# lanl-ansi/RestartSQP

Measured on NVIDIA B200. Metric: QP subproblems/sec, higher is better.
Workload: dtype f64

## Files before the change

restartsqp_b200/csrc/qp_kernel.cuh:

```cuda
#pragma once
#include <cuda_runtime.h>
#include <stdint.h>
#include "tma.cuh"

namespace sqpb200 {

#define QP_EPS 2.221e-16
#define QP_INFTY 1.0e20
#define QP_ZERO 1.0e-25
#define QP_BOUND_RELAX 1.0e4
#define QP_EPS_NUM (-1.0e3 * QP_EPS)
#define QP_EPS_DEN (1.0e3 * QP_EPS)
#define QP_EPS_FLIP (1.0e3 * QP_EPS)
#define QP_EPS_REG (1.0e3 * QP_EPS)
#define QP_EPS_LI (1.0e5 * QP_EPS)

enum { ST_OPTIMAL = 20, ST_INTERNAL = 21, ST_INFEASIBLE = 22, ST_UNBOUNDED = 23, ST_NOTINIT = 25, ST_HOMOTOPY = 28,
       ST_CAPACITY = 31  };
enum { MODE_COLD = 0, MODE_HOT_FIXED = 1, MODE_HOT_VARIED = 2,
       MODE_REINIT = 3  };
enum { FLAG_FLIPPING = 1, FLAG_RAMPING = 2, FLAG_DRIFT = 4, FLAG_KEEP_STATE = 8,
       FLAG_FORCE_GUESS = 16 ,
       FLAG_NO_CARRY = 32 ,
       FLAG_FLIP_AS_HOTSTART = 64  };
// ... 74 lines not shown
extern __shared__ __align__(128) double qp_smem[];

struct MinKey {
    double t;
    int pos;
};
__device__ __forceinline__ bool key_less(double t1, int p1, double t2, int p2) { return t1 < t2 || (t1 == t2 && p1 < p2); }

__device__ __forceinline__ double quot(double x, double d, double ri) {
    const double q0 = x * ri;
    const double r = __fma_rn(-q0, d, x);
    return __fma_rn(r, ri, q0);
}

#define QP_FN __noinline__
#ifndef QP_UNROLL_N
#define QP_UNROLL_N 1
#endif
#define QP_STR_(x) #x
#define QP_STR(x) QP_STR_(x)
#define QP_U1 _Pragma(QP_STR(unroll QP_UNROLL_N))
#ifdef QP_PROFILE
#define PROF_T0 long long prof_t0_ = clock64();
#define PROF_RESET prof_t0_ = clock64();
#define PROF2_T0 long long prof_t2_ = clock64();
#define PROF2_ADD(i) do { long long t_ = clock64(); if (lane == 0 && sA.prof) atomicAdd((unsigned long long*)&sA.prof[i], (unsigned long long)(t_ - prof_t2_)); prof_t2_ = t_; } while (0)
#define PROF_ADD(i) do { long long t_ = clock64(); if (lane == 0 && sA.prof) atomicAdd((unsigned long long*)&sA.prof[i], (unsigned long long)(t_ - prof_t0_)); prof_t0_ = t_; } while (0)
#else
#define PROF_T0
#define PROF_RESET
#define PROF2_T0
#define PROF2_ADD(i) do { } while (0)
#define PROF_ADD(i) do { } while (0)
#endif
enum { PR_STEPDIR = 0, PR_RATIO = 1, PR_STEP = 2, PR_REMOVE = 3, PR_EXTEND = 4, PR_WVEC = 5, PR_ADD = 6, PR_REFAC_W = 7, PR_REFAC_M = 8,
       PR_REFAC_CHOL = 9, PR_DRIFT = 10, PR_ENSURE_LI = 11, PR_RSOLVE = 12, PR_SETUP = 13, PR_EPILOGUE = 14, PR_TOTAL = 15 };

template <int TEAM> struct PatIdx { typedef int type; };
template <> struct PatIdx<32> { typedef short type; };
template <> struct PatIdx<16> { typedef short type; };
template <> struct PatIdx<8> { typedef short type; };
template <int TEAM> __device__ __forceinline__ unsigned team_mask() {
    if (TEAM >= 32) return 0xffffffffu;
    return ((1u << (TEAM & 31)) - 1u) << ((threadIdx.x & 31) & ~(TEAM - 1));
}
__shared__ double* sSlice;
__shared__ int sClusterSize;
__shared__ uint32_t sPhase;
__shared__ __align__(8) uint64_t sFull[3];
__shared__ double sRedT[32];
__shared__ int sRedP[32];

#define QP_CTX                                                                                     \
    const int lane = (TEAM <= 32) ? (int)(threadIdx.x & (TEAM - 1)) : (int)threadIdx.x;            \
    double* const slice = (TEAM <= 32) ? qp_smem + (size_t)(threadIdx.x / TEAM) * sA.slice_doubles : sSlice; \
    int* const hdr = reinterpret_cast<int*>(slice);                                                \
    const int nV = sA.nV, nC = sA.nC, ld = sA.ld, cap = sA.cap;                                    \
    (void)lane; (void)hdr; (void)nV; (void)nC; (void)ld; (void)cap;
#define QP_PAT                                                                                     \
    const pidx* const pat = (TEAM <= 32)                                                           \
        ? reinterpret_cast<const pidx*>(qp_smem + (size_t)(blockDim.x / TEAM) * sA.slice_doubles) \
        : reinterpret_cast<const pidx*>(sA.gpat);

#define V_(name) (slice + sA.o##name)
#define S_(k) (reinterpret_cast<short*>(slice + sA.oS) + (k))
#define sB_ S_(0)
#define FR_ S_(nV)
#define posFR_ S_(2 * nV)
#define sC_ S_(3 * nV)
#define AC_ S_(3 * nV + nC)
#define posAC_ S_(3 * nV + 2 * nC)
#define R_(a_, b_) RT[(a_) * ld + (b_)]
#define T_(i, j) RT[(cap - 1 - (i)) * ld + (j)]
#ifndef QP_DOT_UNROLL_N
#define QP_DOT_UNROLL_N 1
#endif
#define DOT_UNROLL _Pragma("unroll (TEAM <= 32 ? DOT_N_SMALL : 8)")
#define SYNC() do { if (TEAM <= 32) __syncwarp(team_mask<TEAM>()); else __syncthreads(); } while (0)

template <int TEAM>
struct QPT {
    static constexpr int DOT_N_SMALL = QP_DOT_UNROLL_N;
    typedef typename PatIdx<TEAM>::type pidx;
    static __device__ QP_FN void mulH(const double* v, double* out) {
        QP_CTX QP_PAT
        const pidx *Hp = pat + sA.pHp, *Hi = pat + sA.pHi;
        const double* Hv = V_(Hv);
        const bool has_H = sA.has_H && !sA.is_lp;
        const double reg = sA.is_lp ? QP_EPS_REG : 0.0;
        QP_U1 for (int c = lane; c < nV; c += TEAM) {
            double s = 0.0;
            if (has_H) {
                int e1 = Hp[c + 1];
                QP_U1 for (int e = Hp[c]; e < e1; e++) s += Hv[e] * v[Hi[e]];
            }
            if (reg != 0.0) s += reg * v[c];
            out[c] = s;
        }
        SYNC();
    }
    static __device__ QP_FN void mulH_noreg(const double* v, double* out) {
        QP_CTX QP_PAT
        const pidx *Hp = pat + sA.pHp, *Hi = pat + sA.pHi;
        const double* Hv = V_(Hv);
        const bool has_H = sA.has_H && !sA.is_lp;
        QP_U1 for (int c = lane; c < nV; c += TEAM) {
            double s = 0.0;
            if (has_H) {
                int e1 = Hp[c + 1];
                QP_U1 for (int e = Hp[c]; e < e1; e++) s += Hv[e] * v[Hi[e]];
            }
            out[c] = s;
        }
        SYNC();
    }
    static __device__ QP_FN void mulA(const double* v, double* out) {
        QP_CTX QP_PAT
        const pidx *Arp = pat + sA.pArp, *Aci = pat + sA.pAci, *Aperm = pat + sA.pAperm;
        const double* Av = V_(Av);
        QP_U1 for (int r = lane; r < nC; r += TEAM) {
            double s = 0.0;
            int k1 = Arp[r + 1];
            QP_U1 for (int k = Arp[r]; k < k1; k++) s += Av[Aperm[k]] * v[Aci[k]];
            out[r] = s;
        }
        SYNC();
    }
    static __device__ QP_FN void mulAT(const double* yc, double* out) {
        QP_CTX QP_PAT
        const pidx *Ap = pat + sA.pAp, *Ai = pat + sA.pAi;
        const double* Av = V_(Av);
        QP_U1 for (int c = lane; c < nV; c += TEAM) {
            double s = 0.0;
            int e1 = Ap[c + 1];
            QP_U1 for (int e = Ap[c]; e < e1; e++) s += Av[e] * yc[Ai[e]];
            out[c] = s;
        }
        SYNC();
    }
    static __device__ __forceinline__ double A_entry(const pidx* pat, const double* Av, int r, int c) {
        const pidx *Arp = pat + sA.pArp, *Aci = pat + sA.pAci, *Aperm = pat + sA.pAperm;
        double s = 0.0;
        int k1 = Arp[r + 1];
        QP_U1 for (int k = Arp[r]; k < k1; k++)
            if (Aci[k] == c) s += Av[Aperm[k]];
        return s;
    }

    static __device__ __forceinline__ MinKey team_min(double t, int pos) {
        const unsigned tm = team_mask<TEAM>();
        QP_U1 for (int o = (TEAM < 32 ? TEAM : 32) / 2; o > 0; o >>= 1) {
            double t2_ = __shfl_xor_sync(tm, t, o);
            int p2 = __shfl_xor_sync(tm, pos, o);
            if (key_less(t2_, p2, t, pos)) { t = t2_; pos = p2; }
        }
        if (TEAM > 32) {
            __syncthreads();
            if ((threadIdx.x & 31) == 0) { sRedT[threadIdx.x >> 5] = t; sRedP[threadIdx.x >> 5] = pos; }
            __syncthreads();
            t = sRedT[0]; pos = sRedP[0];
            QP_U1 for (int k = 1; k < TEAM / 32; k++)
                if (key_less(sRedT[k], sRedP[k], t, pos)) { t = sRedT[k]; pos = sRedP[k]; }
        }
        MinKey r; r.t = t; r.pos = pos;
        return r;
    }

    static __device__ __forceinline__ void givens(double a_, double b_, double& c, double& s, double& r) {
        if (a_ == 0.0) { c = 1.0; s = 0.0; r = b_; return; }
        double h = sqrt(a_ * a_ + b_ * b_);
        c = b_ / h; s = a_ / h; r = h;
    }

    static __device__ QP_FN void proj_column(int b) {
        QP_CTX
        double *t1 = V_(t1), *t2 = V_(t2);
        const double* Q = V_(Q);
        const short* posFR = posFR_;
        QP_U1 for (int i = lane; i < nV; i += TEAM) { int p = posFR[i]; t1[i] = (p >= 0) ? Q[p * ld + b] : 0.0; }
        SYNC();
        mulH(t1, t2);
    }
    static __device__ QP_FN int recompute_R() {
        QP_CTX
        const int nFR = hdr[0], nAC = hdr[1], nZ = nFR - nAC;
        if (nZ <= 0) return 0;
        double* RT = V_(RT);
        if (sA.is_lp) {
            double sr = sqrt(QP_EPS_REG);
            QP_U1 for (int k = lane; k < nZ * nZ; k += TEAM) { int a_ = k / nZ, b_ = k % nZ; R_(a_, b_) = (a_ == b_) ? sr : 0.0; }
#ifndef QP_EXACT
            if constexpr (TEAM > 32) {
                double* W = V_(W);
                for (int k = lane; k < nZ * 64; k += TEAM) { const int a_ = k >> 6, c_ = k & 63; if (c_ < ld) W[(size_t)a_ * ld + c_] = (c_ == (a_ & 63)) ? 1.0 / sr : 0.0; }
            }
#endif
            SYNC();
            return 0;
        }
        if constexpr (TEAM > 32) return recompute_R_blocked();
        PROF_T0
        {
            QP_PAT
            const double *Q = V_(Q), *Hv = V_(Hv);
            double* Wc = V_(t1);
            const short *FR = FR_, *posFR = posFR_;
            const pidx *Hp = pat + sA.pHp, *Hi = pat + sA.pHi;
            const bool has_H = sA.has_H != 0;
            int CH = sA.nW / nFR;
            if (CH > nZ) CH = nZ;
            QP_U1 for (int b0 = 0; b0 < nZ; b0 += CH) {
                const int cw = (nZ - b0 < CH) ? nZ - b0 : CH;
                QP_U1 for (int e = lane; e < nFR * cw; e += TEAM) {
                    const int p = e / cw, bb = e - p * cw;
                    double s = 0.0;
                    if (has_H) {
                        const int c = FR[p], e1 = Hp[c + 1];
                        QP_U1 for (int h = Hp[c]; h < e1; h++) {
                            const int pr = posFR[Hi[h]];
                            s += Hv[h] * ((pr >= 0) ? Q[pr * ld + b0 + bb] : 0.0);
// ... 1077 lines not shown

    static __device__ QP_FN void constraint_w(int c, double& wz2, double& a2) {
        QP_CTX QP_PAT
        const int nFR = hdr[0], nAC = hdr[1], nZ = nFR - nAC;
        double *a = V_(a), *w = V_(w);
        const double *Q = V_(Q), *Av = V_(Av);
        const short* FR = FR_;
        QP_U1 for (int p = lane; p < nFR; p += TEAM) a[p] = A_entry(pat, Av, c, FR[p]);
        SYNC();
#ifndef QP_EXACT
        if constexpr (TEAM > 32) {
            col_sums_auto(sA.oQ, nFR, 0, nFR, sA.oa, sA.ow, false);
            double s2p = 0.0, z2p = 0.0;
            for (int p = lane; p < nFR; p += TEAM) s2p += a[p] * a[p];
            for (int j = lane; j < nZ; j += TEAM) z2p += w[j] * w[j];
            a2 = team_sum(s2p); wz2 = team_sum(z2p);
            SYNC();
            return;
        }
#endif
        QP_U1 for (int j = lane; j < nFR; j += TEAM) {
            double s = 0.0;
            DOT_UNROLL for (int p = 0; p < nFR; p++) s += Q[p * ld + j] * a[p];
            w[j] = s;
        }
        SYNC();
        double s2 = 0.0, z2 = 0.0;
        DOT_UNROLL for (int p = 0; p < nFR; p++) s2 += a[p] * a[p];
        DOT_UNROLL for (int j = 0; j < nZ; j++) z2 += w[j] * w[j];
        wz2 = z2; a2 = s2;
        SYNC();
    }
    static __device__ QP_FN double rotation_chain(int cnt) {
        QP_CTX
        double *t2 = V_(t2), *t3 = V_(t3);
        const double* w = V_(w);
        QP_U1 for (int j = lane; j + 1 < cnt; j += TEAM) {
            double S = w[0] * w[0];
            bool anyprev = false;
            DOT_UNROLL for (int k = 1; k <= j; k++) { anyprev = anyprev || (w[k - 1] != 0.0); S = S + w[k] * w[k]; }
            const double a = anyprev ? sqrt(S) : w[j];
            if (a == 0.0) { t2[j] = 1.0; t3[j] = 0.0; }
            else { const double h = sqrt(S + w[j + 1] * w[j + 1]); t2[j] = w[j + 1] / h; t3[j] = a / h; }
        }
        double r;
        {
            const int j = cnt - 1;
            double S = w[0] * w[0];
            bool anyprev = false;
            DOT_UNROLL for (int k = 1; k <= j; k++) { anyprev = anyprev || (w[k - 1] != 0.0); S = S + w[k] * w[k]; }
            r = anyprev ? sqrt(S) : w[j];
        }
        SYNC();
        return r;
    }
    static __device__ QP_FN void add_constraint(int c, int status, bool carry_R = false) {
        QP_CTX
        const int nFR = hdr[0], nAC = hdr[1], nZ = nFR - nAC;
        double *Q = V_(Q), *RT = V_(RT);
        const double *t2 = V_(t2), *t3 = V_(t3), *w = V_(w);
        double r = rotation_chain(nZ);
#ifndef QP_EXACT
        if constexpr (TEAM > 32) {
            rot_rows_auto(sA.oQ, nFR, nZ, sA.ot2, sA.ot3);
            if (carry_R) update_R_after_add(nZ);
        } else
#endif
        {
        QP_U1 for (int p = lane; p < nFR; p += TEAM) {
            double* q = Q + p * ld;
            double qa = q[0];
            QP_U1 for (int j = 0; j + 1 < nZ; j++) {
                double cs = t2[j], sn = t3[j], qb = q[j + 1];
                q[j] = cs * qa - sn * qb;
                qa = sn * qa + cs * qb;
            }
            if (nZ > 0) q[nZ - 1] = qa;
        }
        }
        QP_U1 for (int j = lane; j < nFR; j += TEAM) T_(nAC, j) = (j > nZ - 1) ? w[j] : ((j == nZ - 1) ? r : 0.0);
        if (lane == 0) { AC_[nAC] = (short)c; posAC_[c] = (short)nAC; sC_[c] = (short)status; hdr[1] = nAC + 1; }
        SYNC();
    }
    static __device__ QP_FN void remove_constraint(int c) {
        QP_CTX
        const int nFR = hdr[0], nAC = hdr[1];
        double *Q = V_(Q), *RT = V_(RT);
        short *AC = AC_, *posAC = posAC_;
        const int k = posAC[c];
        SYNC();
        QP_U1 for (int i = k + 1; i < nAC; i++) {
            int cL = nFR - 1 - i;
            double cs, sn, r;
            givens(T_(i, cL), T_(i, cL + 1), cs, sn, r);
            SYNC();
            QP_U1 for (int ii = i + lane; ii < nAC; ii += TEAM) {
                double ta = T_(ii, cL), tb = T_(ii, cL + 1);
                T_(ii, cL) = (ii == i) ? 0.0 : cs * ta - sn * tb;
                T_(ii, cL + 1) = sn * ta + cs * tb;
            }
#ifndef QP_EXACT
            if constexpr (TEAM > 32) {
                if (lane == 0) { V_(t2)[i - k - 1] = cs; V_(t3)[i - k - 1] = -sn; }
            } else
#endif
            {
            QP_U1 for (int p = lane; p < nFR; p += TEAM) {
                double qa = Q[p * ld + cL], qb = Q[p * ld + cL + 1];
                Q[p * ld + cL] = cs * qa - sn * qb;
                Q[p * ld + cL + 1] = sn * qa + cs * qb;
            }
            }
            SYNC();
        }
#ifndef QP_EXACT
        if constexpr (TEAM > 32) rot_rows_auto(sA.oQ, nFR, nAC - k, sA.ot2, sA.ot3, nFR - 1 - k, -1);
#endif
        QP_U1 for (int j = lane; j < nFR; j += TEAM)
            QP_U1 for (int i = k + 1; i < nAC; i++) T_(i - 1, j) = T_(i, j);
        SYNC();
        if (lane == 0) {
            QP_U1 for (int i = k + 1; i < nAC; i++) { AC[i - 1] = AC[i]; posAC[AC[i - 1]] = (short)(i - 1); }
            sC_[c] = 0; posAC[c] = -1; hdr[1] = nAC - 1;
        }
        SYNC();
    }
    static __device__ QP_FN double bound_w(int v) {
        QP_CTX
        const int nFR = hdr[0], nAC = hdr[1], nZ = nFR - nAC, p = posFR_[v];
        double* w = V_(w);
        const double* Q = V_(Q);
        QP_U1 for (int j = lane; j < nFR; j += TEAM) w[j] = Q[p * ld + j];
        SYNC();
#ifndef QP_EXACT
        if constexpr (TEAM > 32) {
            double z2p = 0.0;
            for (int j = lane; j < nZ; j += TEAM) z2p += w[j] * w[j];
            const double z2s = team_sum(z2p);
            SYNC();
            return z2s;
        }
#endif
        double z2 = 0.0;
        DOT_UNROLL for (int j = 0; j < nZ; j++) z2 += w[j] * w[j];
        SYNC();
        return z2;
    }
    static __device__ QP_FN void add_bound(int v, int status, bool carry_R = false) {
        QP_CTX
        const int nFR = hdr[0], nAC = hdr[1], nZ = nFR - nAC;
        double *Q = V_(Q), *RT = V_(RT);
        const double *t2 = V_(t2), *t3 = V_(t3);
        short *FR = FR_, *posFR = posFR_;
        const int p = posFR[v];
        rotation_chain(nFR);
#ifndef QP_EXACT
        if constexpr (TEAM > 32) {
            rot_rows_auto(sA.oQ, nFR, nFR, sA.ot2, sA.ot3);
            if (carry_R) update_R_after_add(nZ);
        } else
#endif
        {
        QP_U1 for (int pp = lane; pp < nFR; pp += TEAM) {
            double* q = Q + pp * ld;
            double qa = q[0];
            QP_U1 for (int j = 0; j + 1 < nFR; j++) {
                double cs = t2[j], sn = t3[j], qb = q[j + 1];
                q[j] = cs * qa - sn * qb;
                qa = sn * qa + cs * qb;
            }
            q[nFR - 1] = qa;
        }
        }
        QP_U1 for (int i = lane; i < nAC; i += TEAM) {
            int j0 = nFR - 2 - i; if (j0 < nZ - 1) j0 = nZ - 1; if (j0 < 0) j0 = 0;
            double ta = T_(i, j0);
            QP_U1 for (int j = j0; j + 1 < nFR; j++) {
                double cs = t2[j], sn = t3[j], tb = T_(i, j + 1);
                T_(i, j) = cs * ta - sn * tb;
                ta = sn * ta + cs * tb;
            }
            T_(i, nFR - 1) = ta;
        }
        SYNC();
        const int last = nFR - 1;
        if (p != last) {
            QP_U1 for (int j = lane; j < nFR - 1; j += TEAM) Q[p * ld + j] = Q[last * ld + j];
            if (lane == 0) { short vl = FR[last]; FR[p] = vl; posFR[vl] = (short)p; }
        }
        if (lane == 0) { posFR[v] = -1; sB_[v] = (short)status; hdr[0] = nFR - 1; }
        SYNC();
    }
    static __device__ QP_FN int remove_bound(int v) {
        QP_CTX QP_PAT
        int nFR = hdr[0];
        const int nAC = hdr[1];
        if (nFR + 1 > cap) return 1;
        double *Q = V_(Q), *RT = V_(RT);
        const double* Av = V_(Av);
        const pidx *Ap = pat + sA.pAp, *Ai = pat + sA.pAi;
        const short* AC = AC_;
        SYNC();
        QP_U1 for (int j = lane; j < nFR; j += TEAM) { Q[nFR * ld + j] = 0.0; Q[j * ld + nFR] = 0.0; }
        QP_U1 for (int i = lane; i < nAC; i += TEAM) {
            int r = AC[i];
            double s = 0.0;
            int e1 = Ap[v + 1];
            QP_U1 for (int e = Ap[v]; e < e1; e++)
                if (Ai[e] == r) s += Av[e];
            T_(i, nFR) = s;
        }
        if (lane == 0) { Q[nFR * ld + nFR] = 1.0; FR_[nFR] = (short)v; posFR_[v] = (short)nFR; sB_[v] = 0; hdr[0] = nFR + 1; if (nFR + 1 > hdr[6]) hdr[6] = nFR + 1; }
        nFR++;
        SYNC();
        QP_U1 for (int i = 0; i < nAC; i++) {
            int cL = nFR - 2 - i;
            double cs, sn, r;
            givens(T_(i, cL), T_(i, cL + 1), cs, sn, r);
            SYNC();
            QP_U1 for (int ii = i + lane; ii < nAC; ii += TEAM) {
                double ta = T_(ii, cL), tb = T_(ii, cL + 1);
                T_(ii, cL) = (ii == i) ? 0.0 : cs * ta - sn * tb;
                T_(ii, cL + 1) = sn * ta + cs * tb;
            }
#ifndef QP_EXACT
            if constexpr (TEAM > 32) {
                if (lane == 0) { V_(t2)[i] = cs; V_(t3)[i] = -sn; }
            } else
#endif
            {
            QP_U1 for (int p = lane; p < nFR; p += TEAM) {
                double qa = Q[p * ld + cL], qb = Q[p * ld + cL + 1];
                Q[p * ld + cL] = cs * qa - sn * qb;
                Q[p * ld + cL + 1] = sn * qa + cs * qb;
            }
            }
            SYNC();
        }
#ifndef QP_EXACT
        if constexpr (TEAM > 32) rot_rows_auto(sA.oQ, nFR, nAC + 1, sA.ot2, sA.ot3, nFR - 1, -1);
#endif
        return 0;
    }

    static __device__ QP_FN void solve_T(double* b, double* v) {
        QP_CTX
        const int nFR = hdr[0], nAC = hdr[1];
        const double* RT = V_(RT);
#ifndef QP_EXACT
        if constexpr (TEAM > 32) { solve_T_blocked(b, v); return; }
#endif
        if (TEAM <= 32 && nAC <= TEAM) {
            const bool act = lane < nAC;
            double bk = act ? b[lane] : 0.0;
            const double piv = act ? T_(lane, nFR - 1 - lane) : 1.0, ri = 1.0 / piv;
            QP_U1 for (int i = 0; i < nAC; i++) {
                const int d = nFR - 1 - i;
                const double tkd = (lane > i && act) ? T_(lane, d) : 0.0;
                const double vi = __shfl_sync(team_mask<TEAM>(), quot(bk, piv, ri), i, TEAM <= 32 ? TEAM : 32);
                if (lane == i) v[d] = vi;
                if (lane > i && act) bk -= tkd * vi;
            }
            SYNC();
            return;
        }
        double* rinv = V_(dAx);
        QP_U1 for (int i = lane; i < nAC; i += TEAM) rinv[i] = 1.0 / T_(i, nFR - 1 - i);
        SYNC();
        QP_U1 for (int i = 0; i < nAC; i++) {
            int d = nFR - 1 - i;
            double vi = quot(b[i], T_(i, d), rinv[i]);
            SYNC();
            if (lane == 0) v[d] = vi;
            QP_U1 for (int k = i + 1 + lane; k < nAC; k += TEAM) b[k] -= T_(k, d) * vi;
            SYNC();
        }
    }
    static __device__ QP_FN void solve_Tt(double* r, double* u) {
        QP_CTX
        const int nFR = hdr[0], nAC = hdr[1];
        const double* RT = V_(RT);
#ifndef QP_EXACT
        if constexpr (TEAM > 32) { solve_Tt_blocked(r, u); return; }
#endif
        if (TEAM <= 32 && nAC <= TEAM) {
            const bool act = lane < nAC;
            double rk = act ? r[nFR - 1 - lane] : 0.0;
            const double piv = act ? T_(lane, nFR - 1 - lane) : 1.0, ri = 1.0 / piv;
            QP_U1 for (int i = nAC - 1; i >= 0; i--) {
                const double tik = (lane < i) ? T_(i, nFR - 1 - lane) : 0.0;
                const double ui = __shfl_sync(team_mask<TEAM>(), quot(rk, piv, ri), i, TEAM <= 32 ? TEAM : 32);
                if (lane == i) u[i] = ui;
                if (lane < i) rk -= tik * ui;
            }
            SYNC();
            return;
        }
        double* rinv = V_(dAx);
        QP_U1 for (int i = lane; i < nAC; i += TEAM) rinv[i] = 1.0 / T_(i, nFR - 1 - i);
        SYNC();
        QP_U1 for (int i = nAC - 1; i >= 0; i--) {
            int d = nFR - 1 - i;
            double ui = quot(r[d], T_(i, d), rinv[i]);
            SYNC();
            if (lane == 0) u[i] = ui;
            QP_U1 for (int k = lane; k < i; k += TEAM) { int dk = nFR - 1 - k; r[dk] -= T_(i, dk) * ui; }
            SYNC();
        }
    }

    static __device__ QP_FN void step_direction(const double* dgvec, const double* dxFX, double* dbAC) {
        QP_CTX
        const int nT = nV + nC;
        const int nFR = hdr[0], nAC = hdr[1], nZ = nFR - nAC;
        double *dx = V_(dx), *dy = V_(dy), *t1 = V_(t1), *t2 = V_(t2), *t3 = V_(t3), *yv = V_(yv), *zv = V_(zv);
        const double *Q = V_(Q), *RT = V_(RT);
        const short *sB = sB_, *FR = FR_, *AC = AC_;
        QP_U1 for (int i = lane; i < nV; i += TEAM) dx[i] = (sB[i] != 0) ? dxFX[i] : 0.0;
        SYNC();
        if (nAC > 0) {
            mulA(dx, t2);
            QP_U1 for (int i = lane; i < nAC; i += TEAM) t3[i] = dbAC[i] - t2[AC[i]];
            SYNC();
            solve_T(t3, yv);
#ifndef QP_EXACT
            if constexpr (TEAM > 32) row_sums_auto(sA.oQ, nFR, nZ, nFR, sA.oyv, sA.odx, true, false);
            else
#endif
            {
            QP_U1 for (int p = lane; p < nFR; p += TEAM) {
                double s = 0.0;
                DOT_UNROLL for (int j = nZ; j < nFR; j++) s += Q[p * ld + j] * yv[j];
                dx[FR[p]] = s;
            }
            SYNC();
            }
        }
        if (nZ > 0) {
            mulH(dx, t1);
#ifndef QP_EXACT
            if constexpr (TEAM > 32) {
                for (int p = lane; p < nFR; p += TEAM) { const int v = FR[p]; yv[p] = t1[v] + dgvec[v]; }
                SYNC();
                col_sums_auto(sA.oQ, nFR, 0, nZ, sA.oyv, sA.ozv, true);
            } else
#endif
            {
            QP_U1 for (int j = lane; j < nZ; j += TEAM) {
                double s = 0.0;
                DOT_UNROLL for (int p = 0; p < nFR; p++) { int v = FR[p]; s += Q[p * ld + j] * (t1[v] + dgvec[v]); }
                zv[j] = -s;
            }
            SYNC();
            }
            PROF2_T0
            if constexpr (TEAM > 32) {
                fwd_solve_R_blocked(zv, nZ, -1);
                bwd_solve_R_blocked(zv, nZ);
                PROF2_ADD(PR_RSOLVE);
            } else {
                double* rinv = V_(dy);
                QP_U1 for (int k = lane; k < nZ; k += TEAM) rinv[k] = 1.0 / R_(k, k);
                SYNC();
                QP_U1 for (int k = 0; k < nZ; k++) {
                    double uk = quot(zv[k], R_(k, k), rinv[k]);
                    SYNC();
                    if (lane == 0) zv[k] = uk;
                    QP_U1 for (int i = k + 1 + lane; i < nZ; i += TEAM) zv[i] -= R_(k, i) * uk;
                    SYNC();
                }
                QP_U1 for (int k = nZ - 1; k >= 0; k--) {
                    double zk = quot(zv[k], R_(k, k), rinv[k]);
                    SYNC();
                    if (lane == 0) zv[k] = zk;
                    QP_U1 for (int i = lane; i < k; i += TEAM) zv[i] -= R_(i, k) * zk;
                    SYNC();
                }
                PROF2_ADD(PR_RSOLVE);
            }
#ifndef QP_EXACT
            if constexpr (TEAM > 32) row_sums_auto(sA.oQ, nFR, 0, nZ, sA.ozv, sA.odx, true, true);
            else
#endif
            {
            QP_U1 for (int p = lane; p < nFR; p += TEAM) {
                double s = 0.0;
                DOT_UNROLL for (int j = 0; j < nZ; j++) s += Q[p * ld + j] * zv[j];
                dx[FR[p]] += s;
            }
            SYNC();
            }
        }
        mulH(dx, t1);
        QP_U1 for (int i = lane; i < nV; i += TEAM) t1[i] += dgvec[i];
        QP_U1 for (int i = lane; i < nT; i += TEAM) dy[i] = 0.0;
        SYNC();
        if (nAC > 0) {
#ifndef QP_EXACT
            if constexpr (TEAM > 32) {
                for (int p = lane; p < nFR; p += TEAM) zv[p] = t1[FR[p]];
                SYNC();
                col_sums_auto(sA.oQ, nFR, nZ, nFR, sA.ozv, sA.oyv, false);
            } else
#endif
            {
            QP_U1 for (int j = nZ + lane; j < nFR; j += TEAM) {
                double s = 0.0;
                DOT_UNROLL for (int p = 0; p < nFR; p++) s += Q[p * ld + j] * t1[FR[p]];
                yv[j] = s;
            }
            SYNC();
            }
            solve_Tt(yv, t3);
            QP_U1 for (int i = lane; i < nAC; i += TEAM) dy[nV + AC[i]] = t3[i];
            SYNC();
            mulAT(dy + nV, t2);
            QP_U1 for (int i = lane; i < nV; i += TEAM) if (sB[i] != 0) dy[i] = t1[i] - t2[i];
        } else {
            QP_U1 for (int i = lane; i < nV; i += TEAM) if (sB[i] != 0) dy[i] = t1[i];
        }
        SYNC();
    }

    static __device__ QP_FN void stationarity_gradient() {
        QP_CTX
        double *g = V_(g), *t1 = V_(t1), *t2 = V_(t2);
        const double *x = V_(x), *y = V_(y);
        mulAT(y + nV, t2);
        mulH(x, t1);
        QP_U1 for (int i = lane; i < nV; i += TEAM) g[i] = t2[i] + y[i] - t1[i];
        SYNC();
    }
    static __device__ QP_FN void drift_correction() {
        QP_CTX
        double *x = V_(x), *y = V_(y), *Ax = V_(Ax), *lb = V_(lb), *ub = V_(ub), *lbA = V_(lbA), *ubA = V_(ubA);
        const short *sB = sB_, *sC = sC_;
        mulA(x, Ax);
        QP_U1 for (int i = lane; i < nV; i += TEAM) {
            int s = sB[i]; double xi = x[i];
            if (s < 0) { lb[i] = xi; if (ub[i] < xi) ub[i] = xi; if (y[i] < 0) y[i] = 0.0; }
            else if (s > 0) { ub[i] = xi; if (lb[i] > xi) lb[i] = xi; if (y[i] > 0) y[i] = 0.0; }
            else { if (lb[i] > xi) lb[i] = xi; if (ub[i] < xi) ub[i] = xi; y[i] = 0.0; }
        }
        QP_U1 for (int i = lane; i < nC; i += TEAM) {
            int s = sC[i]; double ax = Ax[i];
            if (s < 0) { lbA[i] = ax; if (ubA[i] < ax) ubA[i] = ax; if (y[nV + i] < 0) y[nV + i] = 0.0; }
            else if (s > 0) { ubA[i] = ax; if (lbA[i] > ax) lbA[i] = ax; if (y[nV + i] > 0) y[nV + i] = 0.0; }
            else { if (lbA[i] > ax) lbA[i] = ax; if (ubA[i] < ax) ubA[i] = ax; y[nV + i] = 0.0; }
        }
        SYNC();
        stationarity_gradient();
    }
    static __device__ QP_FN void ramping() {
        QP_CTX
        double *x = V_(x), *y = V_(y), *Ax = V_(Ax), *lb = V_(lb), *ub = V_(ub), *lbA = V_(lbA), *ubA = V_(ubA);
        const short *sB = sB_, *sC = sC_;
        const int ramp_offset = hdr[2];
        const int nRamp = nV + nC + nC + nV;
        const double r0 = 0.5, r1 = 1.0;
        mulA(x, Ax);
        QP_U1 for (int i = lane; i < nV; i += TEAM) {
            double tP = (double)((i + ramp_offset) % nRamp) / (double)(nRamp - 1);
            double rP = (1.0 - tP) * r0 + tP * r1;
            double tD = (double)((nV + nC + i + ramp_offset) % nRamp) / (double)(nRamp - 1);
            double rD = (1.0 - tD) * r0 + tD * r1;
            double xi = x[i];
            double sca = fabs(xi) > 1.0 ? fabs(xi) : 1.0;
            int s = sB[i];
            if (s >= 0) lb[i] = xi - sca * rP;
            if (s <= 0) ub[i] = xi + sca * rP;
            if (s < 0) { lb[i] = xi; y[i] = rD; }
            if (s > 0) { ub[i] = xi; y[i] = -rD; }
            if (s == 0) y[i] = 0.0;
        }
        QP_U1 for (int i = lane; i < nC; i += TEAM) {
            double tP = (double)((nV + i + ramp_offset) % nRamp) / (double)(nRamp - 1);
            double rP = (1.0 - tP) * r0 + tP * r1;
            double tD = (double)((nV + nC + nV + i + ramp_offset) % nRamp) / (double)(nRamp - 1);
            double rD = (1.0 - tD) * r0 + tD * r1;
            double ax = Ax[i];
            double sca = fabs(ax) > 1.0 ? fabs(ax) : 1.0;
            int s = sC[i];
            if (s >= 0) lbA[i] = ax - sca * rP;
            if (s <= 0) ubA[i] = ax + sca * rP;
            if (s < 0) { lbA[i] = ax; y[nV + i] = rD; }
            if (s > 0) { ubA[i] = ax; y[nV + i] = -rD; }
            if (s == 0) y[nV + i] = 0.0;
        }
        SYNC();
        stationarity_gradient();
        if (lane == 0) hdr[2] = ramp_offset + 1;
        SYNC();
    }

    static __device__ QP_FN int ensure_li(int c, int v, int status) {
        QP_CTX QP_PAT
        const int nFR = hdr[0], nAC = hdr[1], nZ = nFR - nAC;
        double *xiC = V_(zv), *xiB = V_(dx), *yv = V_(yv), *t2 = V_(t2), *t3 = V_(t3), *y = V_(y);
        const double *w = V_(w), *Av = V_(Av);
        const short *sB = sB_, *sC = sC_, *AC = AC_, *posAC = posAC_;
        QP_U1 for (int j = nZ + lane; j < nFR; j += TEAM) yv[j] = w[j];
        SYNC();
        solve_Tt(yv, xiC);
        QP_U1 for (int i = lane; i < nC; i += TEAM) { int p = posAC[i]; t3[i] = (p >= 0) ? xiC[p] : 0.0; }
        SYNC();
        mulAT(t3, t2);
        QP_U1 for (int i = lane; i < nV; i += TEAM) {
            if (sB[i] == 0) { xiB[i] = 0.0; continue; }
            double ai = (c >= 0) ? A_entry(pat, Av, c, i) : 0.0;
            xiB[i] = ai - t2[i];
        }
        SYNC();
        const double sgn = (status < 0) ? 1.0 : -1.0;
        double best = QP_INFTY; int bpos = 0x7fffffff;
        QP_U1 for (int i = lane; i < nAC; i += TEAM) {
            int ci = AC[i]; double xi = sgn * xiC[i], yy = y[nV + ci]; double t = QP_INFTY;
            if (sC[ci] < 0) { if (xi > QP_ZERO && yy >= 0.0) t = yy / xi; }
            else { if (xi < -QP_ZERO && yy <= 0.0) t = yy / xi; }
            if (t < QP_INFTY && key_less(t, i, best, bpos)) { best = t; bpos = i; }
        }
        QP_U1 for (int i = lane; i < nV; i += TEAM) {
            if (sB[i] == 0) continue;
            double xi = sgn * xiB[i], yy = y[i]; double t = QP_INFTY;
            if (sB[i] < 0) { if (xi > QP_ZERO && yy >= 0.0) t = yy / xi; }
            else { if (xi < -QP_ZERO && yy <= 0.0) t = yy / xi; }
            if (t < QP_INFTY && key_less(t, nC + i, best, bpos)) { best = t; bpos = nC + i; }
        }
        MinKey mk = team_min(best, bpos);
        if (mk.pos == 0x7fffffff) return 1;
        const double ymin = mk.t;
        const int kind = mk.pos >= nC ? 1 : 0;
        const int idx = kind ? mk.pos - nC : AC[mk.pos];
        SYNC();
        QP_U1 for (int i = lane; i < nAC; i += TEAM) y[nV + AC[i]] -= ymin * sgn * xiC[i];
        QP_U1 for (int i = lane; i < nV; i += TEAM) if (sB[i] != 0) y[i] -= ymin * sgn * xiB[i];
        SYNC();
        if (lane == 0) {
            if (c >= 0) y[nV + c] = sgn * ymin; else y[v] = sgn * ymin;
            if (kind == 0) y[nV + idx] = 0.0; else y[idx] = 0.0;
        }
        SYNC();
        if (kind == 0) remove_constraint(idx); else if (remove_bound(idx)) return 2;
        return 0;
    }

    static __device__ QP_FN int homotopy(int max_iter, int& iters) {
        QP_CTX
        const int nT = nV + nC;
        const int flags = sA.flags;
        int carried = 0;
        double *x = V_(x), *y = V_(y), *Ax = V_(Ax), *g = V_(g), *lb = V_(lb), *ub = V_(ub), *lbA = V_(lbA), *ubA = V_(ubA);
        double *dx = V_(dx), *dy = V_(dy), *dAx = V_(dAx), *w = V_(w), *a = V_(a);
        const double *gN = V_(gN), *lbN = V_(lbN), *ubN = V_(ubN), *lbAN = V_(lbAN), *ubAN = V_(ubAN);
        short *sB = sB_, *sC = sC_, *AC = AC_;
        iters = 0;
        PROF_T0
        QP_U1 for (int it = 0;; it++) {
            const int nAC = hdr[1];
            QP_U1 for (int i = lane; i < nV; i += TEAM) {
                int s = sB[i];
                w[i] = s < 0 ? (lbN[i] - lb[i]) : (s > 0 ? (ubN[i] - ub[i]) : 0.0);
                a[i] = gN[i] - g[i];
            }
            QP_U1 for (int i = lane; i < nAC; i += TEAM) { int ci = AC[i]; w[nV + i] = sC[ci] < 0 ? (lbAN[ci] - lbA[ci]) : (ubAN[ci] - ubA[ci]); }
            SYNC();
            step_direction(a, w, w + nV);
            mulA(dx, dAx);
            PROF_ADD(PR_STEPDIR);

            double best = 2.0; int bpos = 0x7fffffff;
#define CONSIDER(num, den, pos)                                                                   \
    {                                                                                             \
        double n_ = (num), d_ = (den);                                                            \
        if (d_ >= QP_EPS_DEN && n_ >= QP_EPS_NUM && n_ < d_) {                                    \
            double t_ = n_ / d_;                                                                  \
            if (t_ < 1.0 && key_less(t_, (pos), best, bpos)) { best = t_; bpos = (pos); }         \
        }                                                                                         \
    }
            QP_U1 for (int i = lane; i < nAC; i += TEAM) {
                int ci = AC[i];
                if (sC[ci] < 0) CONSIDER(y[nV + ci], -dy[nV + ci], i) else CONSIDER(-y[nV + ci], dy[nV + ci], i)
            }
            QP_U1 for (int i = lane; i < nV; i += TEAM) {
                int s = sB[i];
                if (s == 0) continue;
                if (s < 0) CONSIDER(y[i], -dy[i], nC + i) else CONSIDER(-y[i], dy[i], nC + i)
            }
            QP_U1 for (int i = lane; i < nC; i += TEAM) {
                if (sC[i] != 0) continue;
                double num = Ax[i] - lbA[i]; if (num < 0) num = 0;
                CONSIDER(num, (lbAN[i] - lbA[i]) - dAx[i], nC + nV + i)
                num = ubA[i] - Ax[i]; if (num < 0) num = 0;
                CONSIDER(num, dAx[i] - (ubAN[i] - ubA[i]), nC + nV + nC + i)
            }
            QP_U1 for (int i = lane; i < nV; i += TEAM) {
                if (sB[i] != 0) continue;
                double num = x[i] - lb[i]; if (num < 0) num = 0;
                CONSIDER(num, (lbN[i] - lb[i]) - dx[i], 2 * nC + nV + nC + i)
                num = ub[i] - x[i]; if (num < 0) num = 0;
                CONSIDER(num, dx[i] - (ubN[i] - ub[i]), 3 * nC + 2 * nV + i)
            }
#undef CONSIDER
            MinKey mk = team_min(best, bpos);
            double tau = 1.0; int bc_idx = -1, bc_isbound = 0, bc_status = 0;
            if (mk.pos != 0x7fffffff) {
                tau = mk.t;
                int p = mk.pos;
                if (p < nC) { bc_idx = AC[p]; bc_isbound = 0; bc_status = 0; }
                else if (p < nC + nV) { bc_idx = p - nC; bc_isbound = 1; bc_status = 0; }
                else if (p < 2 * nC + nV) { bc_idx = p - nC - nV; bc_isbound = 0; bc_status = -1; }
                else if (p < 3 * nC + nV) { bc_idx = p - 2 * nC - nV; bc_isbound = 0; bc_status = 1; }
                else if (p < 3 * nC + 2 * nV) { bc_idx = p - 3 * nC - nV; bc_isbound = 1; bc_status = -1; }
                else { bc_idx = p - 3 * nC - 2 * nV; bc_isbound = 1; bc_status = 1; }
            }
            SYNC();
            PROF_ADD(PR_RATIO);
            if (bc_idx < 0) {
                QP_U1 for (int i = lane; i < nV; i += TEAM) { x[i] += dx[i]; g[i] = gN[i]; lb[i] = lbN[i]; ub[i] = ubN[i]; }
                QP_U1 for (int i = lane; i < nT; i += TEAM) y[i] += dy[i];
                QP_U1 for (int i = lane; i < nC; i += TEAM) { Ax[i] += dAx[i]; lbA[i] = lbAN[i]; ubA[i] = ubAN[i]; }
                SYNC();
                iters = it;
                return ST_OPTIMAL;
            }
            if (it >= max_iter) { iters = it; return ST_HOMOTOPY; }
            if (tau > 0.0) {
                QP_U1 for (int i = lane; i < nV; i += TEAM) {
                    x[i] += tau * dx[i]; g[i] += tau * a[i];
                    lb[i] += tau * (lbN[i] - lb[i]); ub[i] += tau * (ubN[i] - ub[i]);
                }
                QP_U1 for (int i = lane; i < nT; i += TEAM) y[i] += tau * dy[i];
                QP_U1 for (int i = lane; i < nC; i += TEAM) {
                    Ax[i] += tau * dAx[i];
                    lbA[i] += tau * (lbAN[i] - lbA[i]); ubA[i] += tau * (ubAN[i] - ubA[i]);
                }
                SYNC();
            }
            PROF_ADD(PR_STEP);
            if (bc_status == 0) {
                int flipped = 0;
                if (bc_isbound) {
                    int old = sB[bc_idx];
                    SYNC();
                    if (lane == 0) y[bc_idx] = 0.0;
                    SYNC();
                    if (remove_bound(bc_idx)) { iters = it; return ST_CAPACITY; }
                    PROF_ADD(PR_REMOVE);
                    const int ext_ok = extend_R(flags & FLAG_FLIPPING);
                    PROF_ADD(PR_EXTEND);
                    if (!ext_ok) {
// ... 501 lines not shown
```

Measured before the change: 9.722 million.

## Fuse sparse matvecs into consumers and keep Givens removal chain in registers

```diff
diff --git a/restartsqp_b200/csrc/qp_kernel.cuh b/restartsqp_b200/csrc/qp_kernel.cuh
--- a/restartsqp_b200/csrc/qp_kernel.cuh
+++ b/restartsqp_b200/csrc/qp_kernel.cuh
@@ -180,21 +180,35 @@
 struct QPT {
     static constexpr int DOT_N_SMALL = QP_DOT_UNROLL_N;
     typedef typename PatIdx<TEAM>::type pidx;
+    static __device__ __forceinline__ double H_row(const pidx* pat, const double* Hv, const double* v, int c) {
+        const pidx *Hp = pat + sA.pHp, *Hi = pat + sA.pHi;
+        const double reg = sA.is_lp ? QP_EPS_REG : 0.0;
+        double s = 0.0;
+        if (sA.has_H && !sA.is_lp) {
+            int e1 = Hp[c + 1];
+            QP_U1 for (int e = Hp[c]; e < e1; e++) s += Hv[e] * v[Hi[e]];
+        }
+        if (reg != 0.0) s += reg * v[c];
+        return s;
+    }
+    static __device__ __forceinline__ double A_row(const pidx* pat, const double* Av, const double* v, int r) {
+        const pidx *Arp = pat + sA.pArp, *Aci = pat + sA.pAci, *Aperm = pat + sA.pAperm;
+        double s = 0.0;
+        int k1 = Arp[r + 1];
+        QP_U1 for (int k = Arp[r]; k < k1; k++) s += Av[Aperm[k]] * v[Aci[k]];
+        return s;
+    }
+    static __device__ __forceinline__ double AT_col(const pidx* pat, const double* Av, const double* yc, int c) {
+        const pidx *Ap = pat + sA.pAp, *Ai = pat + sA.pAi;
+        double s = 0.0;
+        int e1 = Ap[c + 1];
+        QP_U1 for (int e = Ap[c]; e < e1; e++) s += Av[e] * yc[Ai[e]];
+        return s;
+    }
     static __device__ QP_FN void mulH(const double* v, double* out) {
         QP_CTX QP_PAT
-        const pidx *Hp = pat + sA.pHp, *Hi = pat + sA.pHi;
         const double* Hv = V_(Hv);
-        const bool has_H = sA.has_H && !sA.is_lp;
-        const double reg = sA.is_lp ? QP_EPS_REG : 0.0;
-        QP_U1 for (int c = lane; c < nV; c += TEAM) {
-            double s = 0.0;
-            if (has_H) {
-                int e1 = Hp[c + 1];
-                QP_U1 for (int e = Hp[c]; e < e1; e++) s += Hv[e] * v[Hi[e]];
-            }
-            if (reg != 0.0) s += reg * v[c];
-            out[c] = s;
-        }
+        QP_U1 for (int c = lane; c < nV; c += TEAM) out[c] = H_row(pat, Hv, v, c);
         SYNC();
     }
     static __device__ QP_FN void mulH_noreg(const double* v, double* out) {
@@ -214,26 +228,14 @@
     }
     static __device__ QP_FN void mulA(const double* v, double* out) {
         QP_CTX QP_PAT
-        const pidx *Arp = pat + sA.pArp, *Aci = pat + sA.pAci, *Aperm = pat + sA.pAperm;
         const double* Av = V_(Av);
-        QP_U1 for (int r = lane; r < nC; r += TEAM) {
-            double s = 0.0;
-            int k1 = Arp[r + 1];
-            QP_U1 for (int k = Arp[r]; k < k1; k++) s += Av[Aperm[k]] * v[Aci[k]];
-            out[r] = s;
-        }
+        QP_U1 for (int r = lane; r < nC; r += TEAM) out[r] = A_row(pat, Av, v, r);
         SYNC();
     }
     static __device__ QP_FN void mulAT(const double* yc, double* out) {
         QP_CTX QP_PAT
-        const pidx *Ap = pat + sA.pAp, *Ai = pat + sA.pAi;
         const double* Av = V_(Av);
-        QP_U1 for (int c = lane; c < nV; c += TEAM) {
-            double s = 0.0;
-            int e1 = Ap[c + 1];
-            QP_U1 for (int e = Ap[c]; e < e1; e++) s += Av[e] * yc[Ai[e]];
-            out[c] = s;
-        }
+        QP_U1 for (int c = lane; c < nV; c += TEAM) out[c] = AT_col(pat, Av, yc, c);
         SYNC();
     }
     static __device__ __forceinline__ double A_entry(const pidx* pat, const double* Av, int r, int c) {
@@ -1477,6 +1479,39 @@
         if (lane == 0) { AC_[nAC] = (short)c; posAC_[c] = (short)nAC; sC_[c] = (short)status; hdr[1] = nAC + 1; }
         SYNC();
     }
+    static __device__ QP_FN void removal_chain_regs(int i0, int c0) {
+        QP_CTX
+        const int nFR = hdr[0], nAC = hdr[1];
+        double *Q = V_(Q), *RT = V_(RT), *t2 = V_(t2), *t3 = V_(t3);
+        const unsigned tm = team_mask<TEAM>();
+        constexpr int W = TEAM <= 32 ? TEAM : 32;
+        const bool own = lane >= i0 && lane < nAC;
+        double tb = own ? T_(lane, c0 - i0 + 1) : 0.0;
+        QP_U1 for (int i = i0; i < nAC; i++) {
+            const int cL = c0 - i;
+            const bool act = own && lane >= i;
+            const double ta = act ? T_(lane, cL) : 0.0;
+            double cs, sn, r;
+            givens(__shfl_sync(tm, ta, i, W), __shfl_sync(tm, tb, i, W), cs, sn, r);
+            if (act) {
+                T_(lane, cL + 1) = sn * ta + cs * tb;
+                tb = cs * ta - sn * tb;
+                if (lane == i) { T_(lane, cL) = 0.0; t2[i - i0] = cs; t3[i - i0] = sn; }
+            }
+        }
+        SYNC();
+        QP_U1 for (int p = lane; p < nFR; p += TEAM) {
+            double* q = Q + p * ld;
+            double qb = q[c0 - i0 + 1];
+            QP_U1 for (int i = i0; i < nAC; i++) {
+                const int cL = c0 - i;
+                const double cs = t2[i - i0], sn = t3[i - i0], qa = q[cL];
+                q[cL + 1] = sn * qa + cs * qb;
+                qb = cs * qa - sn * qb;
+            }
+            q[c0 - nAC + 1] = qb;
+        }
+    }
     static __device__ QP_FN void remove_constraint(int c) {
         QP_CTX
         const int nFR = hdr[0], nAC = hdr[1];
@@ -1484,6 +1519,9 @@
         short *AC = AC_, *posAC = posAC_;
         const int k = posAC[c];
         SYNC();
+        if (TEAM <= 32 && nAC <= TEAM) {
+            if (k + 1 < nAC) removal_chain_regs(k + 1, nFR - 1);
+        } else {
         QP_U1 for (int i = k + 1; i < nAC; i++) {
             int cL = nFR - 1 - i;
             double cs, sn, r;
@@ -1507,6 +1545,7 @@
             }
             }
             SYNC();
+        }
         }
 #ifndef QP_EXACT
         if constexpr (TEAM > 32) rot_rows_auto(sA.oQ, nFR, nAC - k, sA.ot2, sA.ot3, nFR - 1 - k, -1);
@@ -1608,6 +1647,10 @@
         if (lane == 0) { Q[nFR * ld + nFR] = 1.0; FR_[nFR] = (short)v; posFR_[v] = (short)nFR; sB_[v] = 0; hdr[0] = nFR + 1; if (nFR + 1 > hdr[6]) hdr[6] = nFR + 1; }
         nFR++;
         SYNC();
+        if (TEAM <= 32 && nAC <= TEAM) {
+            if (nAC > 0) { removal_chain_regs(0, nFR - 2); SYNC(); }
+            return 0;
+        }
         QP_U1 for (int i = 0; i < nAC; i++) {
             int cL = nFR - 2 - i;
             double cs, sn, r;
@@ -1705,17 +1748,16 @@
     }
 
     static __device__ QP_FN void step_direction(const double* dgvec, const double* dxFX, double* dbAC) {
-        QP_CTX
+        QP_CTX QP_PAT
         const int nT = nV + nC;
         const int nFR = hdr[0], nAC = hdr[1], nZ = nFR - nAC;
-        double *dx = V_(dx), *dy = V_(dy), *t1 = V_(t1), *t2 = V_(t2), *t3 = V_(t3), *yv = V_(yv), *zv = V_(zv);
-        const double *Q = V_(Q), *RT = V_(RT);
+        double *dx = V_(dx), *dy = V_(dy), *dAx = V_(dAx), *t1 = V_(t1), *t3 = V_(t3), *yv = V_(yv), *zv = V_(zv);
+        const double *Q = V_(Q), *RT = V_(RT), *Av = V_(Av), *Hv = V_(Hv);
         const short *sB = sB_, *FR = FR_, *AC = AC_;
         QP_U1 for (int i = lane; i < nV; i += TEAM) dx[i] = (sB[i] != 0) ? dxFX[i] : 0.0;
         SYNC();
         if (nAC > 0) {
-            mulA(dx, t2);
-            QP_U1 for (int i = lane; i < nAC; i += TEAM) t3[i] = dbAC[i] - t2[AC[i]];
+            QP_U1 for (int i = lane; i < nAC; i += TEAM) t3[i] = dbAC[i] - A_row(pat, Av, dx, AC[i]);
             SYNC();
             solve_T(t3, yv);
 #ifndef QP_EXACT
@@ -1741,10 +1783,12 @@
             } else
 #endif
             {
+            double* rinv = V_(dy);
             QP_U1 for (int j = lane; j < nZ; j += TEAM) {
                 double s = 0.0;
                 DOT_UNROLL for (int p = 0; p < nFR; p++) { int v = FR[p]; s += Q[p * ld + j] * (t1[v] + dgvec[v]); }
                 zv[j] = -s;
+                rinv[j] = 1.0 / R_(j, j);
             }
             SYNC();
             }
@@ -1754,9 +1798,7 @@
                 bwd_solve_R_blocked(zv, nZ);
                 PROF2_ADD(PR_RSOLVE);
             } else {
-                double* rinv = V_(dy);
-                QP_U1 for (int k = lane; k < nZ; k += TEAM) rinv[k] = 1.0 / R_(k, k);
-                SYNC();
+                const double* rinv = V_(dy);
                 QP_U1 for (int k = 0; k < nZ; k++) {
                     double uk = quot(zv[k], R_(k, k), rinv[k]);
                     SYNC();
@@ -1786,8 +1828,7 @@
             SYNC();
             }
         }
-        mulH(dx, t1);
-        QP_U1 for (int i = lane; i < nV; i += TEAM) t1[i] += dgvec[i];
+        QP_U1 for (int i = lane; i < nV; i += TEAM) t1[i] = H_row(pat, Hv, dx, i) + dgvec[i];
         QP_U1 for (int i = lane; i < nT; i += TEAM) dy[i] = 0.0;
         SYNC();
         if (nAC > 0) {
@@ -1809,51 +1850,56 @@
             solve_Tt(yv, t3);
             QP_U1 for (int i = lane; i < nAC; i += TEAM) dy[nV + AC[i]] = t3[i];
             SYNC();
-            mulAT(dy + nV, t2);
-            QP_U1 for (int i = lane; i < nV; i += TEAM) if (sB[i] != 0) dy[i] = t1[i] - t2[i];
+            QP_U1 for (int i = lane; i < nV; i += TEAM) if (sB[i] != 0) dy[i] = t1[i] - AT_col(pat, Av, dy + nV, i);
         } else {
             QP_U1 for (int i = lane; i < nV; i += TEAM) if (sB[i] != 0) dy[i] = t1[i];
         }
-        SYNC();
-    }
-
+        QP_U1 for (int r = lane; r < nC; r += TEAM) dAx[r] = A_row(pat, Av, dx, r);
+        SYNC();
+    }
+
+    static __device__ QP_FN void stationarity_gradient_tail() {
+        QP_CTX QP_PAT
+        double* g = V_(g);
+        const double *t1 = V_(t1), *y = V_(y), *Av = V_(Av);
+        QP_U1 for (int i = lane; i < nV; i += TEAM) g[i] = AT_col(pat, Av, y + nV, i) + y[i] - t1[i];
+        SYNC();
+    }
     static __device__ QP_FN void stationarity_gradient() {
         QP_CTX
-        double *g = V_(g), *t1 = V_(t1), *t2 = V_(t2);
-        const double *x = V_(x), *y = V_(y);
-        mulAT(y + nV, t2);
-        mulH(x, t1);
-        QP_U1 for (int i = lane; i < nV; i += TEAM) g[i] = t2[i] + y[i] - t1[i];
-        SYNC();
+        mulH(V_(x), V_(t1));
+        stationarity_gradient_tail();
     }
     static __device__ QP_FN void drift_correction() {
-        QP_CTX
-        double *x = V_(x), *y = V_(y), *Ax = V_(Ax), *lb = V_(lb), *ub = V_(ub), *lbA = V_(lbA), *ubA = V_(ubA);
+        QP_CTX QP_PAT
+        double *x = V_(x), *y = V_(y), *Ax = V_(Ax), *lb = V_(lb), *ub = V_(ub), *lbA = V_(lbA), *ubA = V_(ubA), *t1 = V_(t1);
+        const double *Av = V_(Av), *Hv = V_(Hv);
         const short *sB = sB_, *sC = sC_;
-        mulA(x, Ax);
         QP_U1 for (int i = lane; i < nV; i += TEAM) {
             int s = sB[i]; double xi = x[i];
             if (s < 0) { lb[i] = xi; if (ub[i] < xi) ub[i] = xi; if (y[i] < 0) y[i] = 0.0; }
             else if (s > 0) { ub[i] = xi; if (lb[i] > xi) lb[i] = xi; if (y[i] > 0) y[i] = 0.0; }
             else { if (lb[i] > xi) lb[i] = xi; if (ub[i] < xi) ub[i] = xi; y[i] = 0.0; }
+            t1[i] = H_row(pat, Hv, x, i);
         }
         QP_U1 for (int i = lane; i < nC; i += TEAM) {
-            int s = sC[i]; double ax = Ax[i];
+            int s = sC[i]; double ax = A_row(pat, Av, x, i);
+            Ax[i] = ax;
             if (s < 0) { lbA[i] = ax; if (ubA[i] < ax) ubA[i] = ax; if (y[nV + i] < 0) y[nV + i] = 0.0; }
             else if (s > 0) { ubA[i] = ax; if (lbA[i] > ax) lbA[i] = ax; if (y[nV + i] > 0) y[nV + i] = 0.0; }
             else { if (lbA[i] > ax) lbA[i] = ax; if (ubA[i] < ax) ubA[i] = ax; y[nV + i] = 0.0; }
         }
         SYNC();
-        stationarity_gradient();
+        stationarity_gradient_tail();
     }
     static __device__ QP_FN void ramping() {
-        QP_CTX
-        double *x = V_(x), *y = V_(y), *Ax = V_(Ax), *lb = V_(lb), *ub = V_(ub), *lbA = V_(lbA), *ubA = V_(ubA);
+        QP_CTX QP_PAT
+        double *x = V_(x), *y = V_(y), *Ax = V_(Ax), *lb = V_(lb), *ub = V_(ub), *lbA = V_(lbA), *ubA = V_(ubA), *t1 = V_(t1);
+        const double *Av = V_(Av), *Hv = V_(Hv);
         const short *sB = sB_, *sC = sC_;
         const int ramp_offset = hdr[2];
         const int nRamp = nV + nC + nC + nV;
         const double r0 = 0.5, r1 = 1.0;
-        mulA(x, Ax);
         QP_U1 for (int i = lane; i < nV; i += TEAM) {
             double tP = (double)((i + ramp_offset) % nRamp) / (double)(nRamp - 1);
             double rP = (1.0 - tP) * r0 + tP * r1;
@@ -1867,13 +1913,15 @@
             if (s < 0) { lb[i] = xi; y[i] = rD; }
             if (s > 0) { ub[i] = xi; y[i] = -rD; }
             if (s == 0) y[i] = 0.0;
+            t1[i] = H_row(pat, Hv, x, i);
         }
         QP_U1 for (int i = lane; i < nC; i += TEAM) {
             double tP = (double)((nV + i + ramp_offset) % nRamp) / (double)(nRamp - 1);
             double rP = (1.0 - tP) * r0 + tP * r1;
             double tD = (double)((nV + nC + nV + i + ramp_offset) % nRamp) / (double)(nRamp - 1);
             double rD = (1.0 - tD) * r0 + tD * r1;
-            double ax = Ax[i];
+            double ax = A_row(pat, Av, x, i);
+            Ax[i] = ax;
             double sca = fabs(ax) > 1.0 ? fabs(ax) : 1.0;
             int s = sC[i];
             if (s >= 0) lbA[i] = ax - sca * rP;
@@ -1883,29 +1931,25 @@
             if (s == 0) y[nV + i] = 0.0;
         }
         SYNC();
-        stationarity_gradient();
         if (lane == 0) hdr[2] = ramp_offset + 1;
-        SYNC();
+        stationarity_gradient_tail();
     }
 
     static __device__ QP_FN int ensure_li(int c, int v, int status) {
         QP_CTX QP_PAT
         const int nFR = hdr[0], nAC = hdr[1], nZ = nFR - nAC;
-        double *xiC = V_(zv), *xiB = V_(dx), *yv = V_(yv), *t2 = V_(t2), *t3 = V_(t3), *y = V_(y);
-        const double *w = V_(w), *Av = V_(Av);
+        double *xiC = V_(zv), *xiB = V_(dx), *t3 = V_(t3), *y = V_(y), *w = V_(w);
+        const double* Av = V_(Av);
         const short *sB = sB_, *sC = sC_, *AC = AC_, *posAC = posAC_;
-        QP_U1 for (int j = nZ + lane; j < nFR; j += TEAM) yv[j] = w[j];
-        SYNC();
-        solve_Tt(yv, xiC);
+        (void)nZ;
+        solve_Tt(w, xiC);
         QP_U1 for (int i = lane; i < nC; i += TEAM) { int p = posAC[i]; t3[i] = (p >= 0) ? xiC[p] : 0.0; }
         SYNC();
-        mulAT(t3, t2);
         QP_U1 for (int i = lane; i < nV; i += TEAM) {
             if (sB[i] == 0) { xiB[i] = 0.0; continue; }
             double ai = (c >= 0) ? A_entry(pat, Av, c, i) : 0.0;
-            xiB[i] = ai - t2[i];
-        }
-        SYNC();
+            xiB[i] = ai - AT_col(pat, Av, t3, i);
+        }
         const double sgn = (status < 0) ? 1.0 : -1.0;
         double best = QP_INFTY; int bpos = 0x7fffffff;
         QP_U1 for (int i = lane; i < nAC; i += TEAM) {
@@ -1958,9 +2002,7 @@
                 a[i] = gN[i] - g[i];
             }
             QP_U1 for (int i = lane; i < nAC; i += TEAM) { int ci = AC[i]; w[nV + i] = sC[ci] < 0 ? (lbAN[ci] - lbA[ci]) : (ubAN[ci] - ubA[ci]); }
-            SYNC();
             step_direction(a, w, w + nV);
-            mulA(dx, dAx);
             PROF_ADD(PR_STEPDIR);
 
             double best = 2.0; int bpos = 0x7fffffff;
```

New measurement: 10.68 million, median of 6. 1.1x the previous value.
